# liruiluo/VLA-Adapter

Measured on AMD Instinct MI355X. Metric: fine-tune samples/sec (224px img + 32-tok prompt), adapter-only, fwd+bwd+AdamW, higher is better.
Workload: dtype bf16

## Files before the change

### vla_adapter_amd/csrc/attention.hip

```cpp
#include "attn_common.h"
#include "../../include/vla_native.h"

int vla_num_cus();

namespace {

struct AttnP {
  const bf16_t* q; const bf16_t* k; const bf16_t* v; bf16_t* o; float* lse; const unsigned char* kmask;
  long long q_sb, k_sb, v_sb, o_sb; int q_ss, k_ss, v_ss, o_ss;
  int B, Sq, Sk, Hq, Hkv, dh, causal; float scale_log2;
  const bf16_t* dout; bf16_t* dq; bf16_t* dk; bf16_t* dv; float* delta; float scale;
  long long do_sb, dq_sb, dk_sb, dv_sb; int do_ss, dq_ss, dk_ss, dv_ss;
  const float* rope_cos; const float* rope_sin;
  int q_off;
  int dkv_k0;
  int lse_hs;
  int lpt;
};

template <int D, int NT>
struct TileGeo {
  static constexpr int CPR = D / 8;
  static constexpr int NCH = (32 * CPR + NT - 1) / NT;
};
template <int D, int NT>
__device__ __forceinline__ void tile_prefetch(u32x4* __restrict__ v, const bf16_t* src, long long row_stride,
                                              int row0, int nrows, int tid) {
  constexpr int CPR = TileGeo<D, NT>::CPR, NCH = TileGeo<D, NT>::NCH;
#pragma unroll
  for (int i = 0; i < NCH; ++i) {
    const int c = min(tid + i * NT, 32 * CPR - 1);
    const int r = c / CPR, ch = c - r * CPR;
    const int gr = min(row0 + r, nrows - 1);
    v[i] = *reinterpret_cast<const u32x4*>(src + (long long)gr * row_stride + ch * 8);
  }
}
template <int D, int NT, int LD>
__device__ __forceinline__ void tile_store(const u32x4* __restrict__ v, bf16_t* dst, int tid) {
  constexpr int CPR = TileGeo<D, NT>::CPR, NCH = TileGeo<D, NT>::NCH;
#pragma unroll
  for (int i = 0; i < NCH; ++i) {
    const int c = tid + i * NT;
    if (c < 32 * CPR) {
      const int r = c / CPR, ch = c - r * CPR;
      *reinterpret_cast<u32x4*>(dst + r * LD + ch * 8) = v[i];
    }
  }
}

template <int D>
struct Geo {
  static constexpr int DQ = (D + 15) / 16 * 16;
  static constexpr int DV = (D + 31) / 32 * 32;
  static constexpr int LD = DV + 8;
  static constexpr int KS = DQ / 16, DT = DV / 32;
};

template <int D>
__global__ __launch_bounds__(256, (D <= 64 ? 4 : D <= 72 ? 3 : 2)) void attn_fwd_kernel(AttnP p) {
  using G = Geo<D>;
  __shared__ __attribute__((aligned(16))) bf16_t sK[32 * G::LD];
  __shared__ __attribute__((aligned(16))) bf16_t sV[32 * G::LD];
  __shared__ __attribute__((aligned(16))) bf16_t sO[4 * 32 * G::LD];
  const int tid = threadIdx.x, lane = tid & 63, w = tid >> 6, h = lane >> 5;
  const int hq = blockIdx.y, b = p.lpt ? blockIdx.x : blockIdx.z, hkv = hq / (p.Hq / p.Hkv);
  const int qblk = (p.lpt ? (int)(gridDim.z - 1 - blockIdx.z) : (int)blockIdx.x) * 128, q0 = qblk + w * 32;
  const int qi = q0 + (lane & 31);

  lds_zero16(sK, 32 * G::LD * 2, tid, 256);
  lds_zero16(sV, 32 * G::LD * 2, tid, 256);

  bf16x8 qf[G::KS];
  {
    const bf16_t* qp = p.q + (long long)b * p.q_sb + (long long)min(qi, p.Sq - 1) * p.q_ss + hq * D;
#pragma unroll
    for (int ks = 0; ks < G::KS; ++ks) {
      const int d = 16 * ks + 8 * h;
      qf[ks] = (d < D) ? *reinterpret_cast<const bf16x8*>(qp + d) : bf16x8{0, 0, 0, 0, 0, 0, 0, 0};
    }
  }
  f32x16 O[G::DT];
#pragma unroll
  for (int t = 0; t < G::DT; ++t) O[t] = zero16();
  float m_run = -INFINITY, l_run = 0.f;

  const int kend = p.causal ? min(p.Sk, qblk + 128 + p.q_off) : p.Sk;
  const bf16_t* kb = p.k + (long long)b * p.k_sb + hkv * D;
  const bf16_t* vb = p.v + (long long)b * p.v_sb + hkv * D;
  u32x4 rk[TileGeo<D, 256>::NCH], rv[TileGeo<D, 256>::NCH];
  tile_prefetch<D, 256>(rk, kb, p.k_ss, 0, p.Sk, tid);
  tile_prefetch<D, 256>(rv, vb, p.v_ss, 0, p.Sk, tid);
  bool kok_next = (lane & 31) < p.Sk && (!p.kmask || p.kmask[(long long)b * p.Sk + (lane & 31)]);
  for (int k0 = 0; k0 < kend; k0 += 32) {
    __syncthreads();
    tile_store<D, 256, G::LD>(rk, sK, tid);
    tile_store<D, 256, G::LD>(rv, sV, tid);
    const unsigned km = (unsigned)__ballot(kok_next);
    __syncthreads();
    if (k0 + 32 < kend) {
      tile_prefetch<D, 256>(rk, kb, p.k_ss, k0 + 32, p.Sk, tid);
      tile_prefetch<D, 256>(rv, vb, p.v_ss, k0 + 32, p.Sk, tid);
      const int kk = k0 + 32 + (lane & 31);
      kok_next = kk < p.Sk && (!p.kmask || p.kmask[(long long)b * p.Sk + kk]);
    }
    if (p.causal && k0 > q0 + 31 + p.q_off) continue;

    f32x16 S = zero16();
#pragma unroll
    for (int ks = 0; ks < G::KS; ++ks) {
      const bf16x8 kf = *reinterpret_cast<const bf16x8*>(sK + (lane & 31) * G::LD + 16 * ks + 8 * h);
      S = mfma32(kf, qf[ks], S);
    }
#pragma unroll
    for (int r = 0; r < 16; ++r) S[r] *= p.scale_log2;
    if (!(km == 0xffffffffu && (!p.causal || k0 + 31 <= q0 + p.q_off))) {
#pragma unroll
      for (int r = 0; r < 16; ++r) {
        const int kr = acc_row(r, h);
        const bool ok = ((km >> kr) & 1u) && (!p.causal || k0 + kr <= qi + p.q_off);
        S[r] = ok ? S[r] : -INFINITY;
      }
    }
    float mt = -INFINITY;
#pragma unroll
    for (int r = 0; r < 16; ++r) mt = fmaxf(mt, S[r]);
    mt = fmaxf(mt, __shfl_xor(mt, 32, 64));
    const float m_new = fmaxf(m_run, mt);
    const float m_safe = (m_new == -INFINITY) ? 0.f : m_new;
    const float alpha = fexp2(m_run - m_safe);
    float rs = 0.f;
#pragma unroll
    for (int r = 0; r < 16; ++r) {
      S[r] = fexp2(S[r] - m_safe);
      rs += S[r];
    }
    rs += __shfl_xor(rs, 32, 64);
    l_run = l_run * alpha + rs;
    m_run = m_new;
#pragma unroll
    for (int t = 0; t < G::DT; ++t)
#pragma unroll
      for (int r = 0; r < 16; ++r) O[t][r] *= alpha;
#pragma unroll
    for (int s = 0; s < 2; ++s) {
      const bf16x8 pf = pack_acc(S, s);
#pragma unroll
      for (int t = 0; t < G::DT; ++t) O[t] = mfma32(tr_frag(sV, G::LD, s, 32 * t, lane), pf, O[t]);
    }
  }
  const float inv = l_run > 0.f ? 1.f / l_run : 0.f;
  {
    bf16_t* so = sO + w * 32 * G::LD;
#pragma unroll
    for (int t = 0; t < G::DT; ++t)
#pragma unroll
      for (int g = 0; g < 4; ++g) {
        const int d = 32 * t + 8 * g + 4 * h;
        const uint2 o = {pack2(O[t][4 * g] * inv, O[t][4 * g + 1] * inv), pack2(O[t][4 * g + 2] * inv, O[t][4 * g + 3] * inv)};
        *reinterpret_cast<uint2*>(so + (lane & 31) * G::LD + d) = o;
      }
    __builtin_amdgcn_fence(__ATOMIC_RELEASE, "wavefront");
    __builtin_amdgcn_wave_barrier();
    constexpr int CPR = D / 8;
    bf16_t* ob = p.o + (long long)b * p.o_sb + hq * D;
#pragma unroll
    for (int i = 0; i < (32 * CPR + 63) / 64; ++i) {
      const int c = lane + 64 * i, r = c / CPR, ch = c - r * CPR;
      if (c < 32 * CPR && q0 + r < p.Sq)
        *reinterpret_cast<u32x4*>(ob + (long long)(q0 + r) * p.o_ss + ch * 8) = *reinterpret_cast<const u32x4*>(so + r * G::LD + ch * 8);
    }
  }
  if (qi < p.Sq && p.lse && h == 0)
    p.lse[((long long)b * p.Hq + hq) * p.lse_hs + qi] = l_run > 0.f ? (m_run + log2f(l_run)) * 0.6931471805599453f : -INFINITY;
}

template <int D>
__global__ __launch_bounds__(256) void attn_fwd_split_kernel(AttnP p) {
  using G = Geo<D>;
  constexpr int LDO = G::DV + 1;
  extern __shared__ __attribute__((aligned(16))) char smem_split[];
  bf16_t* sV = reinterpret_cast<bf16_t*>(smem_split);
  float* sM = reinterpret_cast<float*>(smem_split + 4 * 32 * G::LD * 2);
  float* sL = sM + 4 * 32;
  float* sO = sL + 4 * 32;
  const int tid = threadIdx.x, lane = tid & 63, w = tid >> 6, h = lane >> 5;
  const int hq = blockIdx.y, b = blockIdx.z, hkv = hq / (p.Hq / p.Hkv);
  const int q0 = blockIdx.x * 32, qi = q0 + (lane & 31);
  bf16_t* sv = sV + w * 32 * G::LD;
  if (D != G::DV) lds_zero16(sv, 32 * G::LD * 2, lane, 64);

  bf16x8 qf[G::KS];
  {
    const bf16_t* qp = p.q + (long long)b * p.q_sb + (long long)min(qi, p.Sq - 1) * p.q_ss + hq * D;
#pragma unroll
    for (int ks = 0; ks < G::KS; ++ks) {
      const int d = 16 * ks + 8 * h;
      qf[ks] = (d < D) ? *reinterpret_cast<const bf16x8*>(qp + d) : bf16x8{0, 0, 0, 0, 0, 0, 0, 0};
    }
  }
  f32x16 O[G::DT];
#pragma unroll
  for (int t = 0; t < G::DT; ++t) O[t] = zero16();
  float m_run = -INFINITY, l_run = 0.f;
  const int kend = p.causal ? min(p.Sk, q0 + 32 + p.q_off) : p.Sk;
  const int ntile = (kend + 31) / 32;
  const bf16_t* kb = p.k + (long long)b * p.k_sb + hkv * D;
  const bf16_t* vb = p.v + (long long)b * p.v_sb + hkv * D;
  for (int kt = w; kt < ntile; kt += 4) {
    const int k0 = kt * 32, kk = k0 + (lane & 31);
    u32x4 rv[TileGeo<D, 64>::NCH];
    tile_prefetch<D, 64>(rv, vb, p.v_ss, k0, p.Sk, lane);
    bf16x8 kf[G::KS];
    {
      const bf16_t* kp = kb + (long long)min(kk, p.Sk - 1) * p.k_ss;
#pragma unroll
      for (int ks = 0; ks < G::KS; ++ks) {
        const int d = 16 * ks + 8 * h;
        kf[ks] = (d < D) ? *reinterpret_cast<const bf16x8*>(kp + d) : bf16x8{0, 0, 0, 0, 0, 0, 0, 0};
      }
    }
    const bool kok = kk < p.Sk && (!p.kmask || p.kmask[(long long)b * p.Sk + kk]);
    const unsigned km = (unsigned)__ballot(kok);
    f32x16 S = zero16();
#pragma unroll
    for (int ks = 0; ks < G::KS; ++ks) S = mfma32(kf[ks], qf[ks], S);
    tile_store<D, 64, G::LD>(rv, sv, lane);
#pragma unroll
    for (int r = 0; r < 16; ++r) S[r] *= p.scale_log2;
    if (!(km == 0xffffffffu && (!p.causal || k0 + 31 <= q0 + p.q_off))) {
#pragma unroll
      for (int r = 0; r < 16; ++r) {
        const int kr = acc_row(r, h);
        const bool ok = ((km >> kr) & 1u) && (!p.causal || k0 + kr <= qi + p.q_off);
        S[r] = ok ? S[r] : -INFINITY;
      }
    }
    float mt = -INFINITY;
#pragma unroll
    for (int r = 0; r < 16; ++r) mt = fmaxf(mt, S[r]);
    mt = fmaxf(mt, __shfl_xor(mt, 32, 64));
    const float m_new = fmaxf(m_run, mt);
    const float m_safe = (m_new == -INFINITY) ? 0.f : m_new;
    const float alpha = fexp2(m_run - m_safe);
    float rs = 0.f;
#pragma unroll
    for (int r = 0; r < 16; ++r) {
      S[r] = fexp2(S[r] - m_safe);
      rs += S[r];
    }
    rs += __shfl_xor(rs, 32, 64);
    l_run = l_run * alpha + rs;
    m_run = m_new;
#pragma unroll
    for (int t = 0; t < G::DT; ++t)
#pragma unroll
      for (int r = 0; r < 16; ++r) O[t][r] *= alpha;
    __builtin_amdgcn_fence(__ATOMIC_RELEASE, "wavefront");
    __builtin_amdgcn_wave_barrier();
#pragma unroll
    for (int s = 0; s < 2; ++s) {
      const bf16x8 pf = pack_acc(S, s);
#pragma unroll
      for (int t = 0; t < G::DT; ++t) O[t] = mfma32(tr_frag(sv, G::LD, s, 32 * t, lane), pf, O[t]);
    }
  }
  if (h == 0) {
    sM[w * 32 + lane] = m_run;
    sL[w * 32 + lane] = l_run;
  }
  {
    float* so = sO + (w * 32 + (lane & 31)) * LDO;
#pragma unroll
    for (int t = 0; t < G::DT; ++t)
#pragma unroll
      for (int g = 0; g < 4; ++g)
#pragma unroll
        for (int j = 0; j < 4; ++j) so[32 * t + 8 * g + 4 * h + j] = O[t][4 * g + j];
  }
  __syncthreads();
  constexpr int CPR = D / 8;
  bf16_t* ob = p.o + (long long)b * p.o_sb + hq * D;
  for (int c = tid; c < 32 * CPR; c += 256) {
    const int q = c / CPR, ch = c - q * CPR;
    if (q0 + q >= p.Sq) continue;
    float mw[4], M = -INFINITY;
#pragma unroll
    for (int ww = 0; ww < 4; ++ww) { mw[ww] = sM[ww * 32 + q]; M = fmaxf(M, mw[ww]); }
    const float Ms = (M == -INFINITY) ? 0.f : M;
    float L = 0.f, f[4];
#pragma unroll
    for (int ww = 0; ww < 4; ++ww) { f[ww] = fexp2(mw[ww] - Ms); L += sL[ww * 32 + q] * f[ww]; }
    const float inv = L > 0.f ? 1.f / L : 0.f;
    float o[8];
#pragma unroll
    for (int e = 0; e < 8; ++e) {
      float a = 0.f;
#pragma unroll
      for (int ww = 0; ww < 4; ++ww) a += sO[(ww * 32 + q) * LDO + ch * 8 + e] * f[ww];
      o[e] = a * inv;
    }
    *reinterpret_cast<u32x4*>(ob + (long long)(q0 + q) * p.o_ss + ch * 8) = u32x4{pack2(o[0], o[1]), pack2(o[2], o[3]), pack2(o[4], o[5]), pack2(o[6], o[7])};
    if (ch == 0 && p.lse) p.lse[((long long)b * p.Hq + hq) * p.lse_hs + q0 + q] = L > 0.f ? (M + log2f(L)) * 0.6931471805599453f : -INFINITY;
  }
}

template <int D>
__global__ __launch_bounds__(256, (D <= 64 ? 3 : 2)) void attn_bwd_dq_kernel(AttnP p) {
  using G = Geo<D>;
  __shared__ __attribute__((aligned(16))) bf16_t sK[32 * G::LD];
  __shared__ __attribute__((aligned(16))) bf16_t sV[32 * G::LD];
  __shared__ __attribute__((aligned(16))) bf16_t sO[4 * 32 * G::LD];
  const int tid = threadIdx.x, lane = tid & 63, w = tid >> 6, h = lane >> 5;
  const int hq = blockIdx.y, b = p.lpt ? blockIdx.x : blockIdx.z, hkv = hq / (p.Hq / p.Hkv);
  const int qblk = (p.lpt ? (int)(gridDim.z - 1 - blockIdx.z) : (int)blockIdx.x) * 128, q0 = qblk + w * 32;
  const int qi = q0 + (lane & 31), qc = min(qi, p.Sq - 1);
  lds_zero16(sK, 32 * G::LD * 2, tid, 256);
  lds_zero16(sV, 32 * G::LD * 2, tid, 256);

  bf16x8 qf[G::KS], dof[G::KS];
  {
    const bf16_t* qp = p.q + (long long)b * p.q_sb + (long long)qc * p.q_ss + hq * D;
    const bf16_t* dp = p.dout + (long long)b * p.do_sb + (long long)qc * p.do_ss + hq * D;
#pragma unroll
    for (int ks = 0; ks < G::KS; ++ks) {
      const int d = 16 * ks + 8 * h;
      const bf16x8 z = {0, 0, 0, 0, 0, 0, 0, 0};
      qf[ks] = (d < D) ? *reinterpret_cast<const bf16x8*>(qp + d) : z;
      dof[ks] = (d < D) ? *reinterpret_cast<const bf16x8*>(dp + d) : z;
    }
  }
  const long long sidx = ((long long)b * p.Hq + hq) * p.Sq + qc;
  const float lse2 = p.lse[((long long)b * p.Hq + hq) * p.lse_hs + qc] * 1.4426950408889634f;
  float delta = 0.f;
  {
    const bf16_t* op = p.o + (long long)b * p.o_sb + (long long)qc * p.o_ss + hq * D;
#pragma unroll
    for (int ks = 0; ks < G::KS; ++ks) {
      const int d = 16 * ks + 8 * h;
      if (d < D) {
        const bf16x8 ov = *reinterpret_cast<const bf16x8*>(op + d);
#pragma unroll
        for (int j = 0; j < 8; ++j) delta += bf2f((bf16_t)ov[j]) * bf2f((bf16_t)dof[ks][j]);
      }
    }
    delta += __shfl_xor(delta, 32, 64);
    if (h == 0 && qi < p.Sq) p.delta[sidx] = delta;
  }
  f32x16 dQ[G::DT];
#pragma unroll
  for (int t = 0; t < G::DT; ++t) dQ[t] = zero16();

  const int kend = p.causal ? min(p.Sk, qblk + 128 + p.q_off) : p.Sk;
  const bf16_t* kb = p.k + (long long)b * p.k_sb + hkv * D;
  const bf16_t* vb = p.v + (long long)b * p.v_sb + hkv * D;
  u32x4 rk[TileGeo<D, 256>::NCH], rv[TileGeo<D, 256>::NCH];
  tile_prefetch<D, 256>(rk, kb, p.k_ss, 0, p.Sk, tid);
  tile_prefetch<D, 256>(rv, vb, p.v_ss, 0, p.Sk, tid);
  bool kok_next = (lane & 31) < p.Sk && (!p.kmask || p.kmask[(long long)b * p.Sk + (lane & 31)]);
  for (int k0 = 0; k0 < kend; k0 += 32) {
    __syncthreads();
    tile_store<D, 256, G::LD>(rk, sK, tid);
    tile_store<D, 256, G::LD>(rv, sV, tid);
    const unsigned km = (unsigned)__ballot(kok_next);
    __syncthreads();
    if (k0 + 32 < kend) {
      tile_prefetch<D, 256>(rk, kb, p.k_ss, k0 + 32, p.Sk, tid);
      tile_prefetch<D, 256>(rv, vb, p.v_ss, k0 + 32, p.Sk, tid);
      const int kk = k0 + 32 + (lane & 31);
      kok_next = kk < p.Sk && (!p.kmask || p.kmask[(long long)b * p.Sk + kk]);
    }
    if (p.causal && k0 > q0 + 31 + p.q_off) continue;
    f32x16 S = zero16(), dP = zero16();
#pragma unroll
    for (int ks = 0; ks < G::KS; ++ks) {
      const bf16x8 kf = *reinterpret_cast<const bf16x8*>(sK + (lane & 31) * G::LD + 16 * ks + 8 * h);
      const bf16x8 vf = *reinterpret_cast<const bf16x8*>(sV + (lane & 31) * G::LD + 16 * ks + 8 * h);
      S = mfma32(kf, qf[ks], S);
      dP = mfma32(vf, dof[ks], dP);
    }
#pragma unroll
    for (int r = 0; r < 16; ++r) {
      const int kr = acc_row(r, h);
      const bool ok = ((km >> kr) & 1u) && (!p.causal || k0 + kr <= qi + p.q_off);
      const float pr = ok ? fexp2(S[r] * p.scale_log2 - lse2) : 0.f;
      S[r] = pr * (dP[r] - delta) * p.scale;
    }
#pragma unroll
    for (int s = 0; s < 2; ++s) {
      const bf16x8 df = pack_acc(S, s);
#pragma unroll
      for (int t = 0; t < G::DT; ++t) dQ[t] = mfma32(tr_frag(sK, G::LD, s, 32 * t, lane), df, dQ[t]);
    }
  }
  if constexpr (G::DT % 2 == 0 && D == 32 * G::DT) {
    if (p.rope_cos) {
      constexpr int HT = G::DT / 2, HALF = D / 2;
#pragma unroll
      for (int t = 0; t < HT; ++t)
#pragma unroll
        for (int g = 0; g < 4; ++g)
#pragma unroll
          for (int j = 0; j < 4; ++j) {
            const int d = 32 * t + 8 * g + 4 * h + j;
            const float c = p.rope_cos[(long long)(qc + p.q_off) * HALF + d], sn = p.rope_sin[(long long)(qc + p.q_off) * HALF + d];
            const float a = dQ[t][4 * g + j], bb = dQ[t + HT][4 * g + j];
            dQ[t][4 * g + j] = a * c + bb * sn;
            dQ[t + HT][4 * g + j] = bb * c - a * sn;
          }
    }
  }
  {
    bf16_t* so = sO + w * 32 * G::LD;
#pragma unroll
    for (int t = 0; t < G::DT; ++t)
#pragma unroll
      for (int g = 0; g < 4; ++g) {
        const int d = 32 * t + 8 * g + 4 * h;
        const uint2 o = {pack2(dQ[t][4 * g], dQ[t][4 * g + 1]), pack2(dQ[t][4 * g + 2], dQ[t][4 * g + 3])};
        *reinterpret_cast<uint2*>(so + (lane & 31) * G::LD + d) = o;
      }
    __builtin_amdgcn_fence(__ATOMIC_RELEASE, "wavefront");
    __builtin_amdgcn_wave_barrier();
    constexpr int CPR = D / 8;
    bf16_t* ob = p.dq + (long long)b * p.dq_sb + hq * D;
#pragma unroll
    for (int i = 0; i < (32 * CPR + 63) / 64; ++i) {
      const int c = lane + 64 * i, r = c / CPR, ch = c - r * CPR;
      if (c < 32 * CPR && q0 + r < p.Sq)
        *reinterpret_cast<u32x4*>(ob + (long long)(q0 + r) * p.dq_ss + ch * 8) = *reinterpret_cast<const u32x4*>(so + r * G::LD + ch * 8);
    }
  }
}

template <int D>
__global__ __launch_bounds__(512) void attn_bwd_dkv_kernel(AttnP p, int grp, int KT) {
  using G = Geo<D>;
  constexpr int TILE = 32 * G::LD;
  constexpr int WAVE_BYTES = 2 * TILE * 2 + 256;
  constexpr int ACC_LD = G::DV + 1;
  extern __shared__ __attribute__((aligned(16))) char smem[];
  const int tid = threadIdx.x, lane = tid & 63, w = tid >> 6, h = lane >> 5;
  const int hh = w % grp, kt = w / grp;
  const int hkv = blockIdx.y, b = p.lpt ? blockIdx.x : blockIdx.z, hq = hkv * grp + hh;
  const int kblk = p.lpt ? blockIdx.z : blockIdx.x;
  const int k0 = p.dkv_k0 + (kblk * KT + kt) * 32;
  const int ki = k0 + (lane & 31), kc = min(ki, p.Sk - 1);
  bf16_t* sQ = reinterpret_cast<bf16_t*>(smem + w * WAVE_BYTES);
  bf16_t* sdO = sQ + TILE;
  float* sLse = reinterpret_cast<float*>(sdO + TILE);
  float* sDelta = sLse + 32;
  lds_zero16(sQ, 2 * TILE * 2, lane, 64);

  constexpr bool KV_LDS = D > 72;
  bf16x8 kf[KV_LDS ? 1 : G::KS], vf[KV_LDS ? 1 : G::KS];
  bf16_t* sKt = reinterpret_cast<bf16_t*>(smem + grp * KT * WAVE_BYTES) + kt * 2 * TILE;
  bf16_t* sVt = sKt + TILE;
  {
    const bf16_t* kp = p.k + (long long)b * p.k_sb + (long long)kc * p.k_ss + hkv * D;
    const bf16_t* vp = p.v + (long long)b * p.v_sb + (long long)kc * p.v_ss + hkv * D;
    if constexpr (KV_LDS) {
      if (hh == 0) {
#pragma unroll
        for (int ks = 0; ks < G::KS; ++ks) {
          const int d = 16 * ks + 8 * h;
          *reinterpret_cast<bf16x8*>(sKt + (lane & 31) * G::LD + d) = *reinterpret_cast<const bf16x8*>(kp + d);
          *reinterpret_cast<bf16x8*>(sVt + (lane & 31) * G::LD + d) = *reinterpret_cast<const bf16x8*>(vp + d);
        }
      }
      __syncthreads();
    } else {
#pragma unroll
      for (int ks = 0; ks < G::KS; ++ks) {
        const int d = 16 * ks + 8 * h;
        const bf16x8 z = {0, 0, 0, 0, 0, 0, 0, 0};
        kf[ks] = (d < D) ? *reinterpret_cast<const bf16x8*>(kp + d) : z;
        vf[ks] = (d < D) ? *reinterpret_cast<const bf16x8*>(vp + d) : z;
      }
    }
  }
  const bool kok = ki < p.Sk && (!p.kmask || p.kmask[(long long)b * p.Sk + kc]);
  f32x16 dK[G::DT], dV[G::DT];
#pragma unroll
  for (int t = 0; t < G::DT; ++t) { dK[t] = zero16(); dV[t] = zero16(); }

  if (k0 < p.Sk) {
    const bf16_t* qb = p.q + (long long)b * p.q_sb + hq * D;
    const bf16_t* db = p.dout + (long long)b * p.do_sb + hq * D;
    const long long sbase = ((long long)b * p.Hq + hq) * p.Sq, lbase = ((long long)b * p.Hq + hq) * p.lse_hs;
    const int qstart = p.causal ? max(k0 - p.q_off, 0) : 0;
    constexpr bool PF = !KV_LDS;
    u32x4 rq[TileGeo<D, 64>::NCH], rdo[TileGeo<D, 64>::NCH];
    if constexpr (PF) {
      tile_prefetch<D, 64>(rq, qb, p.q_ss, qstart, p.Sq, lane);
      tile_prefetch<D, 64>(rdo, db, p.do_ss, qstart, p.Sq, lane);
    }
    float lse_n = 0.f, delta_n = 0.f;
    if (lane < 32) {
      const int qq = min(qstart + lane, p.Sq - 1);
      lse_n = p.lse[lbase + qq];
      delta_n = p.delta[sbase + qq];
    }
    for (int q0 = qstart; q0 < p.Sq; q0 += 32) {
      if constexpr (!PF) {
        tile_prefetch<D, 64>(rq, qb, p.q_ss, q0, p.Sq, lane);
        tile_prefetch<D, 64>(rdo, db, p.do_ss, q0, p.Sq, lane);
      }
      tile_store<D, 64, G::LD>(rq, sQ, lane);
      tile_store<D, 64, G::LD>(rdo, sdO, lane);
      if (lane < 32) {
        sLse[lane] = lse_n * 1.4426950408889634f;
        sDelta[lane] = delta_n;
      }
      if (q0 + 32 < p.Sq) {
        if constexpr (PF) {
          tile_prefetch<D, 64>(rq, qb, p.q_ss, q0 + 32, p.Sq, lane);
          tile_prefetch<D, 64>(rdo, db, p.do_ss, q0 + 32, p.Sq, lane);
        }
        if (lane < 32) {
          const int qq = min(q0 + 32 + lane, p.Sq - 1);
          lse_n = p.lse[lbase + qq];
          delta_n = p.delta[sbase + qq];
        }
      }
      __builtin_amdgcn_fence(__ATOMIC_RELEASE, "wavefront");
      __builtin_amdgcn_wave_barrier();
      f32x16 S = zero16(), dP = zero16();
#pragma unroll
      for (int ks = 0; ks < G::KS; ++ks) {
        const bf16x8 qf = *reinterpret_cast<const bf16x8*>(sQ + (lane & 31) * G::LD + 16 * ks + 8 * h);
        const bf16x8 df = *reinterpret_cast<const bf16x8*>(sdO + (lane & 31) * G::LD + 16 * ks + 8 * h);
        if constexpr (KV_LDS) {
          S = mfma32(qf, *reinterpret_cast<const bf16x8*>(sKt + (lane & 31) * G::LD + 16 * ks + 8 * h), S);
          dP = mfma32(df, *reinterpret_cast<const bf16x8*>(sVt + (lane & 31) * G::LD + 16 * ks + 8 * h), dP);
        } else {
          S = mfma32(qf, kf[ks], S);
          dP = mfma32(df, vf[ks], dP);
        }
      }
      f32x16 dS;
#pragma unroll
      for (int r = 0; r < 16; ++r) {
        const int qr = acc_row(r, h), qq = q0 + qr;
        const bool ok = kok && qq < p.Sq && (!p.causal || ki <= qq + p.q_off);
        const float pr = ok ? fexp2(S[r] * p.scale_log2 - sLse[qr]) : 0.f;
        S[r] = pr;
        dS[r] = pr * (dP[r] - sDelta[qr]) * p.scale;
      }
#pragma unroll
      for (int s = 0; s < 2; ++s) {
        const bf16x8 pf = pack_acc(S, s), dsf = pack_acc(dS, s);
#pragma unroll
        for (int t = 0; t < G::DT; ++t) {
          dV[t] = mfma32(tr_frag(sdO, G::LD, s, 32 * t, lane), pf, dV[t]);
          dK[t] = mfma32(tr_frag(sQ, G::LD, s, 32 * t, lane), dsf, dK[t]);
        }
      }
      __builtin_amdgcn_fence(__ATOMIC_RELEASE, "wavefront");
      __builtin_amdgcn_wave_barrier();
    }
  }
  if (grp > 1) {
    float* part = reinterpret_cast<float*>(smem) + w * (32 * ACC_LD);
#pragma unroll
    for (int pass = 0; pass < 2; ++pass) {
      __syncthreads();
#pragma unroll
      for (int t = 0; t < G::DT; ++t)
#pragma unroll
        for (int r = 0; r < 16; ++r)
          part[(lane & 31) * ACC_LD + 32 * t + acc_row(r, h)] = pass == 0 ? dK[t][r] : dV[t][r];
      __syncthreads();
      bf16_t* outp = pass == 0 ? p.dk : p.dv;
      const long long o_sb = pass == 0 ? p.dk_sb : p.dv_sb;
      const int o_ss = pass == 0 ? p.dk_ss : p.dv_ss;
      for (int i = tid; i < KT * 32 * G::DV; i += blockDim.x) {
        const int kt2 = i / (32 * G::DV), rem = i - kt2 * (32 * G::DV), key = rem / G::DV, d = rem - key * G::DV;
        const int kg = p.dkv_k0 + (kblk * KT + kt2) * 32 + key;
        if (kg < p.Sk && d < D) {
          const float* src = reinterpret_cast<const float*>(smem) + (kt2 * grp) * (32 * ACC_LD) + key * ACC_LD + d;
          float sum = 0.f;
          for (int g = 0; g < grp; ++g) sum += src[g * (32 * ACC_LD)];
          if (pass == 0 && p.rope_cos && (D == 64 || D == 128)) {
            constexpr int HALF = D / 2;
            const float* srp = src + (d < HALF ? HALF : -HALF);
            float other = 0.f;
            for (int g = 0; g < grp; ++g) other += srp[g * (32 * ACC_LD)];
            const float c = p.rope_cos[(long long)kg * HALF + (d & (HALF - 1))], sn = p.rope_sin[(long long)kg * HALF + (d & (HALF - 1))];
            sum = d < HALF ? sum * c + other * sn : sum * c - other * sn;
          }
          outp[(long long)b * o_sb + (long long)(kg - p.dkv_k0) * o_ss + hkv * D + d] = f2bf(sum);
        }
      }
    }
    return;
  }
  if constexpr (G::DT % 2 == 0 && D == 32 * G::DT) {
    if (p.rope_cos) {
      constexpr int HT = G::DT / 2, HALF = D / 2;
#pragma unroll
      for (int t = 0; t < HT; ++t)
#pragma unroll
        for (int g = 0; g < 4; ++g)
#pragma unroll
          for (int j = 0; j < 4; ++j) {
            const int d = 32 * t + 8 * g + 4 * h + j;
            const float c = p.rope_cos[(long long)kc * HALF + d], sn = p.rope_sin[(long long)kc * HALF + d];
            const float a = dK[t][4 * g + j], bb = dK[t + HT][4 * g + j];
            dK[t][4 * g + j] = a * c + bb * sn;
            dK[t + HT][4 * g + j] = bb * c - a * sn;
          }
    }
  }
  if (hh == 0 && ki < p.Sk) {
    bf16_t* okp = p.dk + (long long)b * p.dk_sb + (long long)(ki - p.dkv_k0) * p.dk_ss + hkv * D;
    bf16_t* ovp = p.dv + (long long)b * p.dv_sb + (long long)(ki - p.dkv_k0) * p.dv_ss + hkv * D;
#pragma unroll
    for (int t = 0; t < G::DT; ++t)
#pragma unroll
      for (int g = 0; g < 4; ++g) {
        const int d = 32 * t + 8 * g + 4 * h;
        if (d < D) {
          uint2 a = {pack2(dK[t][4 * g], dK[t][4 * g + 1]), pack2(dK[t][4 * g + 2], dK[t][4 * g + 3])};
          uint2 c = {pack2(dV[t][4 * g], dV[t][4 * g + 1]), pack2(dV[t][4 * g + 2], dV[t][4 * g + 3])};
          *reinterpret_cast<uint2*>(okp + d) = a;
          *reinterpret_cast<uint2*>(ovp + d) = c;
        }
      }
  }
}

int fill(AttnP& p, const vla_attn_desc* d, bool bwd) {
  VLA_REQUIRE(d && d->q && d->k && d->v && d->o, "attn: null tensor");
  VLA_REQUIRE(d->B > 0 && d->Sq > 0 && d->Sk > 0 && d->Hq > 0 && d->Hkv > 0 && d->Hq % d->Hkv == 0, "attn: bad shape");
  VLA_REQUIRE(d->dh == 64 || d->dh == 72 || d->dh == 112 || d->dh == 128, "attn: dh must be 64, 72, 112 or 128");
  VLA_REQUIRE(d->q_ss % 8 == 0 && d->k_ss % 8 == 0 && d->v_ss % 8 == 0 && d->o_ss % 4 == 0, "attn: strides must keep 16-B rows");
  VLA_REQUIRE(d->q_sb % 8 == 0 && d->k_sb % 8 == 0 && d->v_sb % 8 == 0 && d->o_sb % 4 == 0, "attn: batch strides alignment");
  VLA_REQUIRE((((uintptr_t)d->q | (uintptr_t)d->k | (uintptr_t)d->v) & 15) == 0 && ((uintptr_t)d->o & 7) == 0, "attn: alignment");
  VLA_REQUIRE(d->q_ss >= d->Hq * d->dh && d->k_ss >= d->Hkv * d->dh && d->v_ss >= d->Hkv * d->dh, "attn: seq stride < heads*dh");
  p.q = (const bf16_t*)d->q; p.k = (const bf16_t*)d->k; p.v = (const bf16_t*)d->v; p.o = (bf16_t*)d->o;
  p.lse = d->lse; p.kmask = d->kmask;
  p.q_sb = d->q_sb; p.k_sb = d->k_sb; p.v_sb = d->v_sb; p.o_sb = d->o_sb;
  p.q_ss = d->q_ss; p.k_ss = d->k_ss; p.v_ss = d->v_ss; p.o_ss = d->o_ss;
  p.B = d->B; p.Sq = d->Sq; p.Sk = d->Sk; p.Hq = d->Hq; p.Hkv = d->Hkv; p.dh = d->dh; p.causal = d->causal;
  p.scale = d->scale; p.scale_log2 = d->scale * 1.4426950408889634f;
  p.q_off = d->q_off; p.dkv_k0 = d->dkv_k0; p.lse_hs = d->lse_hs > 0 ? d->lse_hs : d->Sq;
  VLA_REQUIRE(d->q_off >= 0 && d->q_off % 32 == 0 && (d->q_off == 0 || (d->causal && d->q_off + d->Sq <= d->Sk)),
              "attn: q_off must be a multiple of 32, causal only, q_off + Sq <= Sk");
  VLA_REQUIRE(d->dkv_k0 >= 0 && d->dkv_k0 % 32 == 0 && d->dkv_k0 < d->Sk && p.lse_hs >= d->Sq, "attn: bad dkv_k0 / lse_hs");
  if (bwd) {
    VLA_REQUIRE(d->dout && d->dq && d->dk && d->dv && d->delta && d->lse, "attn_bwd: null tensor");
    VLA_REQUIRE(d->do_ss % 8 == 0 && d->do_sb % 8 == 0 && ((uintptr_t)d->dout & 15) == 0, "attn_bwd: dout alignment");
    VLA_REQUIRE(d->dq_ss % 4 == 0 && d->dk_ss % 4 == 0 && d->dv_ss % 4 == 0 && d->dq_sb % 4 == 0 && d->dk_sb % 4 == 0 &&
                d->dv_sb % 4 == 0 && (((uintptr_t)d->dq | (uintptr_t)d->dk | (uintptr_t)d->dv) & 7) == 0, "attn_bwd: grad alignment");
    VLA_REQUIRE(d->o_ss % 8 == 0 && d->o_sb % 8 == 0 && ((uintptr_t)d->o & 15) == 0, "attn_bwd: o must allow 16-B row loads");
    p.dout = (const bf16_t*)d->dout; p.dq = (bf16_t*)d->dq; p.dk = (bf16_t*)d->dk; p.dv = (bf16_t*)d->dv; p.delta = d->delta;
    p.do_sb = d->do_sb; p.dq_sb = d->dq_sb; p.dk_sb = d->dk_sb; p.dv_sb = d->dv_sb;
    p.do_ss = d->do_ss; p.dq_ss = d->dq_ss; p.dk_ss = d->dk_ss; p.dv_ss = d->dv_ss;
    p.rope_cos = d->rope_cos; p.rope_sin = d->rope_sin;
    if (d->rope_cos) VLA_REQUIRE(d->rope_sin && (d->dh == 64 || d->dh == 128) && d->Sq + d->q_off == d->Sk, "attn_bwd: fused inverse RoPE needs dh 64 or 128 (tables f32 [Sk, dh/2])");
  }
  return VLA_OK;
}

}

extern "C" int vla_attn_fwd(void* stream, const vla_attn_desc* d) {
  AttnP p{};
  int rc = fill(p, d, false);
  if (rc) return rc;
  dim3 grid((p.Sq + 127) / 128, p.Hq, p.B);
  hipStream_t st = (hipStream_t)stream;
  if (vla_gemm_latency_hint(-1) > 0 && (p.dh == 64 || p.dh == 72) && (long long)grid.x * grid.y * grid.z * 2 <= vla_num_cus()) {
    const dim3 g2((p.Sq + 31) / 32, p.Hq, p.B);
    const int dv = (p.dh + 31) / 32 * 32;
    const size_t lds = (size_t)4 * 32 * (dv + 8) * 2 + 2 * 4 * 32 * 4 + (size_t)4 * 32 * (dv + 1) * 4;
    if (int rc = vla_lds_limit<attn_fwd_split_kernel<72>>(96 * 1024, "attn_fwd_split_kernel")) return rc;
    if (p.dh == 64) hipLaunchKernelGGL(attn_fwd_split_kernel<64>, g2, dim3(256), lds, st, p);
    else hipLaunchKernelGGL(attn_fwd_split_kernel<72>, g2, dim3(256), lds, st, p);
    VLA_CHECK_LAUNCH("attn_fwd(split)");
    return VLA_OK;
  }
  if (p.causal && grid.x > 1 && grid.x <= 65535) { p.lpt = 1; grid = dim3(p.B, p.Hq, grid.x); }
  switch (p.dh) {
    case 64: hipLaunchKernelGGL(attn_fwd_kernel<64>, grid, dim3(256), 0, st, p); break;
    case 72: hipLaunchKernelGGL(attn_fwd_kernel<72>, grid, dim3(256), 0, st, p); break;
    case 112: hipLaunchKernelGGL(attn_fwd_kernel<112>, grid, dim3(256), 0, st, p); break;
    default: hipLaunchKernelGGL(attn_fwd_kernel<128>, grid, dim3(256), 0, st, p); break;
  }
  VLA_CHECK_LAUNCH("attn_fwd");
  return VLA_OK;
}

extern "C" int vla_attn_bwd(void* stream, const vla_attn_desc* d) {
  AttnP p{};
  int rc = fill(p, d, true);
  if (rc) return rc;
  VLA_REQUIRE(p.dh == 64 || p.dh == 72 || p.dh == 128, "attn_bwd: dh 64, 72 or 128 only");
  VLA_REQUIRE(p.dh == 64 || p.dh == 128 || !p.rope_cos, "attn_bwd: the fused inverse RoPE needs head dim 64 or 128 (apply vla_rope_half with sign -1 otherwise)");
  hipStream_t st = (hipStream_t)stream;
  const int grp = p.Hq / p.Hkv;
  VLA_REQUIRE(grp <= 8, "attn_bwd: at most 8 query heads per kv head");
  const int KT = grp >= 4 ? 1 : 4 / grp;
  dim3 gq((p.Sq + 127) / 128, p.Hq, p.B), gk((p.Sk - p.dkv_k0 + 32 * KT - 1) / (32 * KT), p.Hkv, p.B);
  if (p.causal && gq.x <= 65535 && gk.x <= 65535 && (gq.x > 1 || gk.x > 1)) {
    p.lpt = 1;
    gq = dim3(p.B, p.Hq, gq.x);
    gk = dim3(p.B, p.Hkv, gk.x);
  }
  const int ld = ((p.dh + 31) / 32 * 32 + 8);
  const size_t lds = (size_t)grp * KT * (2 * 32 * ld * 2 + 256) + (p.dh > 72 ? (size_t)KT * 2 * 32 * ld * 2 : 0);
  VLA_REQUIRE(lds <= 160 * 1024, "attn_bwd: LDS budget exceeded");
  rc = p.dh == 64 ? vla_lds_limit<attn_bwd_dkv_kernel<64>>(160 * 1024, "attn_bwd_dkv_kernel")
       : p.dh == 72 ? vla_lds_limit<attn_bwd_dkv_kernel<72>>(160 * 1024, "attn_bwd_dkv_kernel")
                    : vla_lds_limit<attn_bwd_dkv_kernel<128>>(160 * 1024, "attn_bwd_dkv_kernel");
  if (rc) return rc;
  if (p.dh == 64) {
    hipLaunchKernelGGL(attn_bwd_dq_kernel<64>, gq, dim3(256), 0, st, p);
    hipLaunchKernelGGL(attn_bwd_dkv_kernel<64>, gk, dim3(64 * grp * KT), lds, st, p, grp, KT);
  } else if (p.dh == 72) {
    hipLaunchKernelGGL(attn_bwd_dq_kernel<72>, gq, dim3(256), 0, st, p);
    hipLaunchKernelGGL(attn_bwd_dkv_kernel<72>, gk, dim3(64 * grp * KT), lds, st, p, grp, KT);
  } else {
    hipLaunchKernelGGL(attn_bwd_dq_kernel<128>, gq, dim3(256), 0, st, p);
    hipLaunchKernelGGL(attn_bwd_dkv_kernel<128>, gk, dim3(64 * grp * KT), lds, st, p, grp, KT);
  }
  VLA_CHECK_LAUNCH("attn_bwd");
  return VLA_OK;
}
```

Baseline: 1364.

## Double-buffer 64-row K/V tiles in attention fwd and bwd-dq kernels

The forward and dQ-backward attention kernels now stage 64 K/V rows per iteration into a ping-pong LDS ring instead of 32 rows into a single buffer. That halves the block-wide barriers per key range, since each iteration needs one __syncthreads instead of two, and it lets the next tile's register prefetch overlap compute on the current image. The output staging buffer sO now aliases the ring, and the LDS zero-fill runs only when head dims need padding. In exchange, LDS per block grows and the prefetch register arrays double in size, which may reduce occupancy or raise register pressure.

```diff
diff --git a/vla_adapter_amd/csrc/attention.hip b/vla_adapter_amd/csrc/attention.hip
--- a/vla_adapter_amd/csrc/attention.hip
+++ b/vla_adapter_amd/csrc/attention.hip
@@ -18,30 +18,30 @@
   int lpt;
 };
 
-template <int D, int NT>
+template <int D, int NT, int ROWS = 32>
 struct TileGeo {
   static constexpr int CPR = D / 8;
-  static constexpr int NCH = (32 * CPR + NT - 1) / NT;
+  static constexpr int NCH = (ROWS * CPR + NT - 1) / NT;
 };
-template <int D, int NT>
+template <int D, int NT, int ROWS = 32>
 __device__ __forceinline__ void tile_prefetch(u32x4* __restrict__ v, const bf16_t* src, long long row_stride,
                                               int row0, int nrows, int tid) {
-  constexpr int CPR = TileGeo<D, NT>::CPR, NCH = TileGeo<D, NT>::NCH;
+  constexpr int CPR = TileGeo<D, NT, ROWS>::CPR, NCH = TileGeo<D, NT, ROWS>::NCH;
 #pragma unroll
   for (int i = 0; i < NCH; ++i) {
-    const int c = min(tid + i * NT, 32 * CPR - 1);
+    const int c = min(tid + i * NT, ROWS * CPR - 1);
     const int r = c / CPR, ch = c - r * CPR;
     const int gr = min(row0 + r, nrows - 1);
     v[i] = *reinterpret_cast<const u32x4*>(src + (long long)gr * row_stride + ch * 8);
   }
 }
-template <int D, int NT, int LD>
+template <int D, int NT, int LD, int ROWS = 32>
 __device__ __forceinline__ void tile_store(const u32x4* __restrict__ v, bf16_t* dst, int tid) {
-  constexpr int CPR = TileGeo<D, NT>::CPR, NCH = TileGeo<D, NT>::NCH;
+  constexpr int CPR = TileGeo<D, NT, ROWS>::CPR, NCH = TileGeo<D, NT, ROWS>::NCH;
 #pragma unroll
   for (int i = 0; i < NCH; ++i) {
     const int c = tid + i * NT;
-    if (c < 32 * CPR) {
+    if (c < ROWS * CPR) {
       const int r = c / CPR, ch = c - r * CPR;
       *reinterpret_cast<u32x4*>(dst + r * LD + ch * 8) = v[i];
     }
@@ -54,22 +54,22 @@
   static constexpr int DV = (D + 31) / 32 * 32;
   static constexpr int LD = DV + 8;
   static constexpr int KS = DQ / 16, DT = DV / 32;
+  static constexpr int IMG = 64 * LD;
+  static constexpr int RING = 2 * 2 * IMG;
+  static constexpr bool PADS_READ = DQ != D || DV != D;
 };
 
 template <int D>
 __global__ __launch_bounds__(256, (D <= 64 ? 4 : D <= 72 ? 3 : 2)) void attn_fwd_kernel(AttnP p) {
   using G = Geo<D>;
-  __shared__ __attribute__((aligned(16))) bf16_t sK[32 * G::LD];
-  __shared__ __attribute__((aligned(16))) bf16_t sV[32 * G::LD];
-  __shared__ __attribute__((aligned(16))) bf16_t sO[4 * 32 * G::LD];
+  __shared__ __attribute__((aligned(16))) bf16_t ring[G::RING];
+  bf16_t* const sO = ring;
+  static_assert(4 * 32 * G::LD <= G::RING, "sO aliases the ring");
   const int tid = threadIdx.x, lane = tid & 63, w = tid >> 6, h = lane >> 5;
   const int hq = blockIdx.y, b = p.lpt ? blockIdx.x : blockIdx.z, hkv = hq / (p.Hq / p.Hkv);
   const int qblk = (p.lpt ? (int)(gridDim.z - 1 - blockIdx.z) : (int)blockIdx.x) * 128, q0 = qblk + w * 32;
   const int qi = q0 + (lane & 31);
 
-  lds_zero16(sK, 32 * G::LD * 2, tid, 256);
-  lds_zero16(sV, 32 * G::LD * 2, tid, 256);
-
   bf16x8 qf[G::KS];
   {
     const bf16_t* qp = p.q + (long long)b * p.q_sb + (long long)min(qi, p.Sq - 1) * p.q_ss + hq * D;
@@ -87,67 +87,82 @@
   const int kend = p.causal ? min(p.Sk, qblk + 128 + p.q_off) : p.Sk;
   const bf16_t* kb = p.k + (long long)b * p.k_sb + hkv * D;
   const bf16_t* vb = p.v + (long long)b * p.v_sb + hkv * D;
-  u32x4 rk[TileGeo<D, 256>::NCH], rv[TileGeo<D, 256>::NCH];
-  tile_prefetch<D, 256>(rk, kb, p.k_ss, 0, p.Sk, tid);
-  tile_prefetch<D, 256>(rv, vb, p.v_ss, 0, p.Sk, tid);
-  bool kok_next = (lane & 31) < p.Sk && (!p.kmask || p.kmask[(long long)b * p.Sk + (lane & 31)]);
-  for (int k0 = 0; k0 < kend; k0 += 32) {
+  u32x4 rk[TileGeo<D, 256, 64>::NCH], rv[TileGeo<D, 256, 64>::NCH];
+  tile_prefetch<D, 256, 64>(rk, kb, p.k_ss, 0, p.Sk, tid);
+  tile_prefetch<D, 256, 64>(rv, vb, p.v_ss, 0, p.Sk, tid);
+  bool kok_next = lane < p.Sk && (!p.kmask || p.kmask[(long long)b * p.Sk + lane]);
+  if constexpr (G::PADS_READ) {
+    lds_zero16(ring, G::RING * 2, tid, 256);
     __syncthreads();
-    tile_store<D, 256, G::LD>(rk, sK, tid);
-    tile_store<D, 256, G::LD>(rv, sV, tid);
-    const unsigned km = (unsigned)__ballot(kok_next);
+  }
+  for (int k0 = 0, img = 0; k0 < kend; k0 += 64, img ^= 1) {
+    bf16_t* const sK = ring + img * (2 * G::IMG);
+    bf16_t* const sV = sK + G::IMG;
+    tile_store<D, 256, G::LD, 64>(rk, sK, tid);
+    tile_store<D, 256, G::LD, 64>(rv, sV, tid);
+    const unsigned long long km2 = __ballot(kok_next);
     __syncthreads();
-    if (k0 + 32 < kend) {
-      tile_prefetch<D, 256>(rk, kb, p.k_ss, k0 + 32, p.Sk, tid);
-      tile_prefetch<D, 256>(rv, vb, p.v_ss, k0 + 32, p.Sk, tid);
-      const int kk = k0 + 32 + (lane & 31);
+    if (k0 + 64 < kend) {
+      tile_prefetch<D, 256, 64>(rk, kb, p.k_ss, k0 + 64, p.Sk, tid);
+      tile_prefetch<D, 256, 64>(rv, vb, p.v_ss, k0 + 64, p.Sk, tid);
+      const int kk = k0 + 64 + lane;
       kok_next = kk < p.Sk && (!p.kmask || p.kmask[(long long)b * p.Sk + kk]);
     }
-    if (p.causal && k0 > q0 + 31 + p.q_off) continue;
-
-    f32x16 S = zero16();
-#pragma unroll
-    for (int ks = 0; ks < G::KS; ++ks) {
-      const bf16x8 kf = *reinterpret_cast<const bf16x8*>(sK + (lane & 31) * G::LD + 16 * ks + 8 * h);
-      S = mfma32(kf, qf[ks], S);
-    }
-#pragma unroll
-    for (int r = 0; r < 16; ++r) S[r] *= p.scale_log2;
-    if (!(km == 0xffffffffu && (!p.causal || k0 + 31 <= q0 + p.q_off))) {
-#pragma unroll
-      for (int r = 0; r < 16; ++r) {
-        const int kr = acc_row(r, h);
-        const bool ok = ((km >> kr) & 1u) && (!p.causal || k0 + kr <= qi + p.q_off);
-        S[r] = ok ? S[r] : -INFINITY;
-      }
-    }
-    float mt = -INFINITY;
-#pragma unroll
-    for (int r = 0; r < 16; ++r) mt = fmaxf(mt, S[r]);
-    mt = fmaxf(mt, __shfl_xor(mt, 32, 64));
-    const float m_new = fmaxf(m_run, mt);
-    const float m_safe = (m_new == -INFINITY) ? 0.f : m_new;
-    const float alpha = fexp2(m_run - m_safe);
-    float rs = 0.f;
-#pragma unroll
-    for (int r = 0; r < 16; ++r) {
-      S[r] = fexp2(S[r] - m_safe);
-      rs += S[r];
-    }
-    rs += __shfl_xor(rs, 32, 64);
-    l_run = l_run * alpha + rs;
-    m_run = m_new;
-#pragma unroll
-    for (int t = 0; t < G::DT; ++t)
-#pragma unroll
-      for (int r = 0; r < 16; ++r) O[t][r] *= alpha;
-#pragma unroll
-    for (int s = 0; s < 2; ++s) {
-      const bf16x8 pf = pack_acc(S, s);
-#pragma unroll
-      for (int t = 0; t < G::DT; ++t) O[t] = mfma32(tr_frag(sV, G::LD, s, 32 * t, lane), pf, O[t]);
-    }
-  }
+#pragma unroll 1
+    for (int tt = 0; tt < 2; ++tt) {
+      const int kt = k0 + 32 * tt;
+      if (kt < kend && !(p.causal && kt > q0 + 31 + p.q_off)) {
+        const unsigned km = (unsigned)(km2 >> (32 * tt));
+        const bf16_t* const tK = sK + 32 * tt * G::LD;
+        const bf16_t* const tV = sV + 32 * tt * G::LD;
+
+        f32x16 S = zero16();
+#pragma unroll
+        for (int ks = 0; ks < G::KS; ++ks) {
+          const bf16x8 kf = *reinterpret_cast<const bf16x8*>(tK + (lane & 31) * G::LD + 16 * ks + 8 * h);
+          S = mfma32(kf, qf[ks], S);
+        }
+#pragma unroll
+        for (int r = 0; r < 16; ++r) S[r] *= p.scale_log2;
+        if (!(km == 0xffffffffu && (!p.causal || kt + 31 <= q0 + p.q_off))) {
+          const unsigned kmh = km >> (4 * h);
+#pragma unroll
+          for (int r = 0; r < 16; ++r) {
+            const int kr = acc_row(r, h);
+            const bool ok = ((kmh >> acc_row(r, 0)) & 1u) && (!p.causal || kt + kr <= qi + p.q_off);
+            S[r] = ok ? S[r] : -INFINITY;
+          }
+        }
+        float mt = -INFINITY;
+#pragma unroll
+        for (int r = 0; r < 16; ++r) mt = fmaxf(mt, S[r]);
+        mt = fmaxf(mt, __shfl_xor(mt, 32, 64));
+        const float m_new = fmaxf(m_run, mt);
+        const float m_safe = (m_new == -INFINITY) ? 0.f : m_new;
+        const float alpha = fexp2(m_run - m_safe);
+        float rs = 0.f;
+#pragma unroll
+        for (int r = 0; r < 16; ++r) {
+          S[r] = fexp2(S[r] - m_safe);
+          rs += S[r];
+        }
+        rs += __shfl_xor(rs, 32, 64);
+        l_run = l_run * alpha + rs;
+        m_run = m_new;
+#pragma unroll
+        for (int t = 0; t < G::DT; ++t)
+#pragma unroll
+          for (int r = 0; r < 16; ++r) O[t][r] *= alpha;
+#pragma unroll
+        for (int s = 0; s < 2; ++s) {
+          const bf16x8 pf = pack_acc(S, s);
+#pragma unroll
+          for (int t = 0; t < G::DT; ++t) O[t] = mfma32(tr_frag(tV, G::LD, s, 32 * t, lane), pf, O[t]);
+        }
+      }
+    }
+  }
+  __syncthreads();
   const float inv = l_run > 0.f ? 1.f / l_run : 0.f;
   {
     bf16_t* so = sO + w * 32 * G::LD;
@@ -307,15 +322,13 @@
 template <int D>
 __global__ __launch_bounds__(256, (D <= 64 ? 3 : 2)) void attn_bwd_dq_kernel(AttnP p) {
   using G = Geo<D>;
-  __shared__ __attribute__((aligned(16))) bf16_t sK[32 * G::LD];
-  __shared__ __attribute__((aligned(16))) bf16_t sV[32 * G::LD];
-  __shared__ __attribute__((aligned(16))) bf16_t sO[4 * 32 * G::LD];
+  __shared__ __attribute__((aligned(16))) bf16_t ring[G::RING];
+  bf16_t* const sO = ring;
+  static_assert(4 * 32 * G::LD <= G::RING, "sO aliases the ring");
   const int tid = threadIdx.x, lane = tid & 63, w = tid >> 6, h = lane >> 5;
   const int hq = blockIdx.y, b = p.lpt ? blockIdx.x : blockIdx.z, hkv = hq / (p.Hq / p.Hkv);
   const int qblk = (p.lpt ? (int)(gridDim.z - 1 - blockIdx.z) : (int)blockIdx.x) * 128, q0 = qblk + w * 32;
   const int qi = q0 + (lane & 31), qc = min(qi, p.Sq - 1);
-  lds_zero16(sK, 32 * G::LD * 2, tid, 256);
-  lds_zero16(sV, 32 * G::LD * 2, tid, 256);
 
   bf16x8 qf[G::KS], dof[G::KS];
   {
@@ -353,45 +366,60 @@
   const int kend = p.causal ? min(p.Sk, qblk + 128 + p.q_off) : p.Sk;
   const bf16_t* kb = p.k + (long long)b * p.k_sb + hkv * D;
   const bf16_t* vb = p.v + (long long)b * p.v_sb + hkv * D;
-  u32x4 rk[TileGeo<D, 256>::NCH], rv[TileGeo<D, 256>::NCH];
-  tile_prefetch<D, 256>(rk, kb, p.k_ss, 0, p.Sk, tid);
-  tile_prefetch<D, 256>(rv, vb, p.v_ss, 0, p.Sk, tid);
-  bool kok_next = (lane & 31) < p.Sk && (!p.kmask || p.kmask[(long long)b * p.Sk + (lane & 31)]);
-  for (int k0 = 0; k0 < kend; k0 += 32) {
+  u32x4 rk[TileGeo<D, 256, 64>::NCH], rv[TileGeo<D, 256, 64>::NCH];
+  tile_prefetch<D, 256, 64>(rk, kb, p.k_ss, 0, p.Sk, tid);
+  tile_prefetch<D, 256, 64>(rv, vb, p.v_ss, 0, p.Sk, tid);
+  bool kok_next = lane < p.Sk && (!p.kmask || p.kmask[(long long)b * p.Sk + lane]);
+  if constexpr (G::PADS_READ) {
+    lds_zero16(ring, G::RING * 2, tid, 256);
     __syncthreads();
-    tile_store<D, 256, G::LD>(rk, sK, tid);
-    tile_store<D, 256, G::LD>(rv, sV, tid);
-    const unsigned km = (unsigned)__ballot(kok_next);
+  }
+  for (int k0 = 0, img = 0; k0 < kend; k0 += 64, img ^= 1) {
+    bf16_t* const sK = ring + img * (2 * G::IMG);
+    bf16_t* const sV = sK + G::IMG;
+    tile_store<D, 256, G::LD, 64>(rk, sK, tid);
+    tile_store<D, 256, G::LD, 64>(rv, sV, tid);
+    const unsigned long long km2 = __ballot(kok_next);
     __syncthreads();
-    if (k0 + 32 < kend) {
-      tile_prefetch<D, 256>(rk, kb, p.k_ss, k0 + 32, p.Sk, tid);
-      tile_prefetch<D, 256>(rv, vb, p.v_ss, k0 + 32, p.Sk, tid);
-      const int kk = k0 + 32 + (lane & 31);
+    if (k0 + 64 < kend) {
+      tile_prefetch<D, 256, 64>(rk, kb, p.k_ss, k0 + 64, p.Sk, tid);
+      tile_prefetch<D, 256, 64>(rv, vb, p.v_ss, k0 + 64, p.Sk, tid);
+      const int kk = k0 + 64 + lane;
       kok_next = kk < p.Sk && (!p.kmask || p.kmask[(long long)b * p.Sk + kk]);
     }
-    if (p.causal && k0 > q0 + 31 + p.q_off) continue;
-    f32x16 S = zero16(), dP = zero16();
-#pragma unroll
-    for (int ks = 0; ks < G::KS; ++ks) {
-      const bf16x8 kf = *reinterpret_cast<const bf16x8*>(sK + (lane & 31) * G::LD + 16 * ks + 8 * h);
-      const bf16x8 vf = *reinterpret_cast<const bf16x8*>(sV + (lane & 31) * G::LD + 16 * ks + 8 * h);
-      S = mfma32(kf, qf[ks], S);
-      dP = mfma32(vf, dof[ks], dP);
-    }
-#pragma unroll
-    for (int r = 0; r < 16; ++r) {
-      const int kr = acc_row(r, h);
-      const bool ok = ((km >> kr) & 1u) && (!p.causal || k0 + kr <= qi + p.q_off);
-      const float pr = ok ? fexp2(S[r] * p.scale_log2 - lse2) : 0.f;
-      S[r] = pr * (dP[r] - delta) * p.scale;
-    }
-#pragma unroll
-    for (int s = 0; s < 2; ++s) {
-      const bf16x8 df = pack_acc(S, s);
-#pragma unroll
-      for (int t = 0; t < G::DT; ++t) dQ[t] = mfma32(tr_frag(sK, G::LD, s, 32 * t, lane), df, dQ[t]);
-    }
-  }
+#pragma unroll 1
+    for (int tt = 0; tt < 2; ++tt) {
+      const int kt = k0 + 32 * tt;
+      if (kt < kend && !(p.causal && kt > q0 + 31 + p.q_off)) {
+        const unsigned km = (unsigned)(km2 >> (32 * tt));
+        const unsigned kmh = km >> (4 * h);
+        const bf16_t* const tK = sK + 32 * tt * G::LD;
+        const bf16_t* const tV = sV + 32 * tt * G::LD;
+        f32x16 S = zero16(), dP = zero16();
+#pragma unroll
+        for (int ks = 0; ks < G::KS; ++ks) {
+          const bf16x8 kf = *reinterpret_cast<const bf16x8*>(tK + (lane & 31) * G::LD + 16 * ks + 8 * h);
+          const bf16x8 vf = *reinterpret_cast<const bf16x8*>(tV + (lane & 31) * G::LD + 16 * ks + 8 * h);
+          S = mfma32(kf, qf[ks], S);
+          dP = mfma32(vf, dof[ks], dP);
+        }
+#pragma unroll
+        for (int r = 0; r < 16; ++r) {
+          const int kr = acc_row(r, h);
+          const bool ok = ((kmh >> acc_row(r, 0)) & 1u) && (!p.causal || kt + kr <= qi + p.q_off);
+          const float pr = ok ? fexp2(S[r] * p.scale_log2 - lse2) : 0.f;
+          S[r] = pr * (dP[r] - delta) * p.scale;
+        }
+#pragma unroll
+        for (int s = 0; s < 2; ++s) {
+          const bf16x8 df = pack_acc(S, s);
+#pragma unroll
+          for (int t = 0; t < G::DT; ++t) dQ[t] = mfma32(tr_frag(tK, G::LD, s, 32 * t, lane), df, dQ[t]);
+        }
+      }
+    }
+  }
+  __syncthreads();
   if constexpr (G::DT % 2 == 0 && D == 32 * G::DT) {
     if (p.rope_cos) {
       constexpr int HT = G::DT / 2, HALF = D / 2;
```

After: 1368, median of 6. About the same (+0.3%).
